# zhaodong-liu/GRAM

Measured on AMD Instinct MI355X. Metric: users/sec @ beam=20 top-20 gen, Beauty T5-base; Recall@5 parity, higher is better.
Workload: dtype f16x3

## Files before the change

gram_amd/csrc/enc_attn.hip:

```cpp
#include "common.h"
#include "prof.h"

#ifndef GRAM_ENC_ABL
#define GRAM_ENC_ABL 0
#endif

namespace {

__device__ __forceinline__ int kswz(int row, int chunk) { return row * 128 + ((chunk ^ ((row >> 1) & 7)) << 4); }
__device__ __forceinline__ int vtswz(int d, int key) { return d * 256 + ((((key >> 3) ^ (d & 15))) << 4) + (key & 7) * 2; }

template <int NKS, int S, bool ROWS>
__global__ __launch_bounds__(256) void enc_attn_kernel(const p16* __restrict__ qkv, const float* __restrict__ bias,
                                                       const uint8_t* __restrict__ mask, p16* __restrict__ out, int H,
                                                       long qkv_pstride, const int64_t* __restrict__ ids) {
  constexpr int L = 32 * NKS;
  using T = SplitTab<S>;
  extern __shared__ __attribute__((aligned(16))) char smem[];
  char* ks = smem;
  char* vts = smem + S * 128 * 128;
  float* bias_s = reinterpret_cast<float*>(smem + S * 2 * 128 * 128);
  float* mask_s = bias_s + 4 * 256;

  const int h = blockIdx.x, p = blockIdx.y;
  const int tid = threadIdx.x, lane = tid & 63, wave = tid >> 6;
  const int inner = H * 64;
  const size_t rs = (size_t)3 * inner;
  const p16* base = qkv + (ROWS ? (size_t)0 : (size_t)p * L * rs) + h * 64;
  long kvid[ROWS ? NKS : 1], qid[2];
  float bias_early = 0.f;
  uint32_t mask_early = 1;
  if constexpr (ROWS) {
    const int64_t* pid = ids + (size_t)p * L;
#pragma unroll
    for (int it = 0; it < NKS; ++it) kvid[it] = pid[(tid + it * 256) >> 3];
#pragma unroll
    for (int nt = 0; nt < 2; ++nt) qid[nt] = wave * 32 < L ? pid[wave * 32 + 16 * nt + (lane & 15)] : 0;
    if (tid < 255) bias_early = bias[h * 255 + tid];
    if (tid < L) mask_early = mask[(size_t)p * L + tid];
    asm volatile("" : "+v"(bias_early), "+v"(mask_early));
  }

#pragma unroll
  for (int pc = 0; pc < S; ++pc) {
    p16x8 kv[NKS], vv[NKS];
#pragma unroll
    for (int it = 0; it < NKS; ++it) {
      const int i = tid + it * 256, row = i >> 3, c = i & 7;
      const p16* src = base + pc * qkv_pstride + (size_t)(ROWS ? kvid[it] : row) * rs + c * 8;
      if constexpr ((GRAM_ENC_ABL & 8) != 0) {
        kv[it] = zero_bf16x8();
        vv[it] = zero_bf16x8();
        asm volatile("" : "+v"(kv[it]), "+v"(vv[it]));
      } else {
        kv[it] = ld_stream_b128(src + inner);
        vv[it] = ld_stream_b128(src + 2 * inner);
      }
    }
#pragma unroll
    for (int it = 0; it < NKS; ++it) {
      const int i = tid + it * 256, row = i >> 3, c = i & 7;
      *reinterpret_cast<p16x8*>(ks + pc * 128 * 128 + kswz(row, c)) = kv[it];
      if constexpr ((GRAM_ENC_ABL & 16) != 0) {
        *reinterpret_cast<p16x8*>(vts + pc * 64 * 256 + kswz(row, c)) = vv[it];
      } else {
#pragma unroll
        for (int e = 0; e < 8; ++e) *reinterpret_cast<p16*>(vts + pc * 64 * 256 + vtswz(c * 8 + e, row)) = vv[it][e];
      }
    }
  }
  if (tid < 255) {
    const float bv = ROWS ? bias_early : bias[h * 255 + tid];
#pragma unroll
    for (int r = 0; r < 4; ++r)
      if (tid >= r) bias_s[r * 256 + tid - r] = bv;
  }
  bool key_masked = false;
  if (tid < L) {
    key_masked = (ROWS ? mask_early : mask[(size_t)p * L + tid]) == 0;
    mask_s[tid] = key_masked ? 1.f : 0.f;
  }
  const bool any_masked = __syncthreads_or(key_masked) != 0;

  const int q0 = wave * 32;
  if (q0 >= L) return;
  const int c = lane & 15, g = lane >> 4;

  p16x8 qf[S][2][2];
#pragma unroll
  for (int pc = 0; pc < S; ++pc)
#pragma unroll
    for (int nt = 0; nt < 2; ++nt)
#pragma unroll
      for (int kd = 0; kd < 2; ++kd)
        if constexpr ((GRAM_ENC_ABL & 64) != 0) {
          qf[pc][nt][kd] = zero_bf16x8();
          asm volatile("" : "+v"(qf[pc][nt][kd]));
        } else {
          qf[pc][nt][kd] = ld_stream_b128(base + pc * qkv_pstride + (size_t)(ROWS ? qid[nt] : q0 + 16 * nt + c) * rs + 32 * kd + 8 * g);
        }

  f32x4 s[NKS][2][2];
#pragma unroll
  for (int k2 = 0; k2 < NKS; ++k2)
#pragma unroll
    for (int t = 0; t < 2; ++t) {
      const int key = 32 * k2 + 8 * (c >> 2) + 4 * t + (c & 3);
      p16x8 kf[S][2];
#pragma unroll
      for (int pc = 0; pc < S; ++pc) {
        kf[pc][0] = *reinterpret_cast<const p16x8*>(ks + pc * 128 * 128 + kswz(key, g));
        kf[pc][1] = *reinterpret_cast<const p16x8*>(ks + pc * 128 * 128 + kswz(key, 4 + g));
      }
#pragma unroll
      for (int nt = 0; nt < 2; ++nt) {
        const int idx0 = 32 * k2 + 8 * g + 4 * t + 127 - (q0 + 16 * nt + c), r = idx0 & 3;
        f32x4 a = *reinterpret_cast<const f32x4*>(bias_s + r * 256 + (idx0 - r));
        if constexpr ((GRAM_ENC_ABL & 1) != 0) {
          a[0] += (float)kf[0][0][0] + (float)qf[0][nt][0][0];
        } else {
#pragma unroll
          for (int pr = 0; pr < T::NP; ++pr) {
            a = mfma16(kf[T::A[pr]][0], qf[T::B[pr]][nt][0], a);
            a = mfma16(kf[T::A[pr]][1], qf[T::B[pr]][nt][1], a);
          }
        }
        s[k2][t][nt] = a;
      }
    }

  gram_sync();

  float mxq[2], l[2] = {0.f, 0.f};
#pragma unroll
  for (int nt = 0; nt < 2; ++nt) {
    float mx = GRAM_FMIN;
#pragma unroll
    for (int k2 = 0; k2 < NKS; ++k2)
#pragma unroll
      for (int t = 0; t < 2; ++t)
#pragma unroll
        for (int j = 0; j < 4; ++j) {
          float v = s[k2][t][nt][j];
          if (any_masked) {
            v = (mask_s[32 * k2 + 8 * g + 4 * t + j] != 0.f) ? GRAM_FMIN : v;
            s[k2][t][nt][j] = v;
          }
          mx = fmaxf(mx, v);
        }
    mx = fmaxf(mx, __shfl_xor(mx, 16, 64));
    mx = fmaxf(mx, __shfl_xor(mx, 32, 64));
    mxq[nt] = mx;
  }

  f32x4 o[4][2];
#pragma unroll
  for (int mt = 0; mt < 4; ++mt)
#pragma unroll
    for (int nt = 0; nt < 2; ++nt) o[mt][nt] = (f32x4){0.f, 0.f, 0.f, 0.f};
#pragma unroll
  for (int k2 = 0; k2 < NKS; ++k2) {
    p16x8 pf[S][2];
#pragma unroll
    for (int nt = 0; nt < 2; ++nt) {
      if constexpr ((GRAM_ENC_ABL & 2) != 0) {
        float t = 0.f;
#pragma unroll
        for (int tt = 0; tt < 2; ++tt)
#pragma unroll
          for (int j = 0; j < 4; ++j) t += s[k2][tt][nt][j];
        l[nt] += t;
        const uint32_t wv = __float_as_uint(t) & 0x3c003c00u;
        pf[0][nt] = __builtin_bit_cast(p16x8, make_uint4(wv, wv, wv, wv));
        if constexpr (S == 2) pf[S - 1][nt] = pf[0][nt];
      } else if constexpr (S == 2) {
        uint32_t w[2][4];
#pragma unroll
        for (int t = 0; t < 2; ++t)
#pragma unroll
          for (int j = 0; j < 4; j += 2) {
            const float e0 = __expf(s[k2][t][nt][j] - mxq[nt]), e1 = __expf(s[k2][t][nt][j + 1] - mxq[nt]);
            l[nt] += e0;
            l[nt] += e1;
            split2_pair(e0, e1, w[0][2 * t + (j >> 1)], w[1][2 * t + (j >> 1)]);
          }
        pf[0][nt] = __builtin_bit_cast(p16x8, make_uint4(w[0][0], w[0][1], w[0][2], w[0][3]));
        pf[1][nt] = __builtin_bit_cast(p16x8, make_uint4(w[1][0], w[1][1], w[1][2], w[1][3]));
      } else {
#pragma unroll
        for (int t = 0; t < 2; ++t)
#pragma unroll
          for (int j = 0; j < 4; ++j) {
            const float e = __expf(s[k2][t][nt][j] - mxq[nt]);
            l[nt] += e;
            pf[0][nt][4 * t + j] = (p16)e;
          }
      }
    }
#pragma unroll
    for (int mt = 0; mt < 4; ++mt) {
      const int d = 16 * mt + c;
      p16x8 vf[S];
#pragma unroll
      for (int pc = 0; pc < S; ++pc) vf[pc] = *reinterpret_cast<const p16x8*>(vts + pc * 64 * 256 + vtswz(d, 32 * k2 + 8 * g));
#pragma unroll
      for (int nt = 0; nt < 2; ++nt)
#pragma unroll
        for (int pr = 0; pr < T::NP; ++pr) {
          if constexpr ((GRAM_ENC_ABL & 4) != 0) o[mt][nt][0] += (float)vf[T::A[pr]][0] + (float)pf[T::B[pr]][nt][0];
          else o[mt][nt] = mfma16(vf[T::A[pr]], pf[T::B[pr]][nt], o[mt][nt]);
        }
    }
  }

  constexpr int RB = 128 * S, CPR = RB / 16;
  char* stage = ks + wave * (32 * RB);
#pragma unroll
  for (int nt = 0; nt < 2; ++nt) {
    float lt = l[nt];
    lt += __shfl_xor(lt, 16, 64);
    lt += __shfl_xor(lt, 32, 64);
    const float inv_l = 1.f / lt;
    const int ql = 16 * nt + c;
#pragma unroll
    for (int mt = 0; mt < 4; ++mt) {
      const f32x4 v = o[mt][nt] * inv_l;
      if constexpr (S == 2) {
        uint2 hi, lo;
        split2x4(v, hi, lo);
        const int ch = (mt >> 1) * 8 + (mt & 1) * 2 + (g >> 1);
        *reinterpret_cast<uint2*>(stage + ql * RB + (((ch) ^ (ql & 15)) << 4) + (g & 1) * 8) = hi;
        *reinterpret_cast<uint2*>(stage + ql * RB + (((ch + 4) ^ (ql & 15)) << 4) + (g & 1) * 8) = lo;
      } else {
        p16x4 r;
#pragma unroll
        for (int j = 0; j < 4; ++j) r[j] = (p16)v[j];
        const int ch = 2 * mt + (g >> 1);
        *reinterpret_cast<p16x4*>(stage + ql * RB + ((ch ^ (ql & 7)) << 4) + (g & 1) * 8) = r;
      }
    }
  }
  __builtin_amdgcn_wave_barrier();
  asm volatile("s_waitcnt lgkmcnt(0)" ::: "memory");
  char* obase = reinterpret_cast<char*>(out) + (((size_t)p * L + q0) * inner * S + (size_t)h * 64 * S) * sizeof(p16);
#pragma unroll
  for (int it = 0; it < RB / 32; ++it) {
    const int row = it * (64 / CPR) + lane / CPR, chunk = lane % CPR;
    const uint4 val = *reinterpret_cast<const uint4*>(stage + row * RB + ((chunk ^ (row & (CPR - 1))) << 4));
    if (!(GRAM_ENC_ABL & 32) || val.x == 0x12345678u)
      *reinterpret_cast<uint4*>(obase + (size_t)row * inner * S * sizeof(p16) + chunk * 16) = val;
  }
}

template <int S, bool ROWS>
int launch_enc(const void* qkv, const int64_t* ids, const float* bias, const uint8_t* mask, void* out, int P, int L, int H,
               long qkv_pstride, hipStream_t st) {
  const dim3 grid(H, P), block(256);
  constexpr int smem = S * 2 * 128 * 128 + (4 * 256 + 128) * 4;
  static bool attr_set = false;
  if (!attr_set && smem > 48 * 1024) {
    hipError_t e = hipFuncSetAttribute(reinterpret_cast<const void*>(enc_attn_kernel<1, S, ROWS>), hipFuncAttributeMaxDynamicSharedMemorySize, smem);
    if (e == hipSuccess) e = hipFuncSetAttribute(reinterpret_cast<const void*>(enc_attn_kernel<2, S, ROWS>), hipFuncAttributeMaxDynamicSharedMemorySize, smem);
    if (e == hipSuccess) e = hipFuncSetAttribute(reinterpret_cast<const void*>(enc_attn_kernel<3, S, ROWS>), hipFuncAttributeMaxDynamicSharedMemorySize, smem);
    if (e == hipSuccess) e = hipFuncSetAttribute(reinterpret_cast<const void*>(enc_attn_kernel<4, S, ROWS>), hipFuncAttributeMaxDynamicSharedMemorySize, smem);
    if (e != hipSuccess) return (int)e;
    attr_set = true;
  }
  switch (L / 32) {
    case 1: hipLaunchKernelGGL((enc_attn_kernel<1, S, ROWS>), grid, block, smem, st, (const p16*)qkv, bias, mask, (p16*)out, H, qkv_pstride, ids); break;
    case 2: hipLaunchKernelGGL((enc_attn_kernel<2, S, ROWS>), grid, block, smem, st, (const p16*)qkv, bias, mask, (p16*)out, H, qkv_pstride, ids); break;
    case 3: hipLaunchKernelGGL((enc_attn_kernel<3, S, ROWS>), grid, block, smem, st, (const p16*)qkv, bias, mask, (p16*)out, H, qkv_pstride, ids); break;
    default: hipLaunchKernelGGL((enc_attn_kernel<4, S, ROWS>), grid, block, smem, st, (const p16*)qkv, bias, mask, (p16*)out, H, qkv_pstride, ids); break;
  }
  GRAM_CHECK_LAUNCH();
  return 0;
}

}

extern "C" int gram_enc_self_attn(const void* qkv, const float* bias, const uint8_t* mask, void* out, int P, int L, int H,
                                  void* stream) {
  return gram_enc_self_attn_split(qkv, bias, mask, out, P, L, H, 1, 0, stream);
}

extern "C" int gram_enc_self_attn_split(const void* qkv, const float* bias, const uint8_t* mask, void* out, int P, int L, int H,
                                        int pieces, int64_t qkv_pstride, void* stream) {
  if (P < 1 || H < 1 || L < 32 || L > GRAM_MAX_PASSAGE_LEN || (L & 31) || pieces < 1 || pieces > GRAM_MAX_PIECES) return GRAM_E_ARG;
  if (pieces > 1 && qkv_pstride < (int64_t)P * L * 3 * H * 64) return GRAM_E_ARG;
  hipStream_t st = (hipStream_t)stream;
  gram_prof::Scope prof(GRAM_K_ENC_ATTN, st, 4.0 * P * H * L * L * 64 * (pieces == 2 ? 3 : 1));
  if (pieces == 2) return launch_enc<2, false>(qkv, nullptr, bias, mask, out, P, L, H, qkv_pstride, st);
  return launch_enc<1, false>(qkv, nullptr, bias, mask, out, P, L, H, qkv_pstride, st);
}

extern "C" int gram_enc_self_attn_rows_split(const void* qkv_table, const int64_t* ids, const float* bias, const uint8_t* mask,
                                             void* out, int P, int L, int H, int pieces, int64_t qkv_pstride, void* stream) {
  if (P < 1 || H < 1 || L < 32 || L > GRAM_MAX_PASSAGE_LEN || (L & 31) || pieces < 1 || pieces > GRAM_MAX_PIECES || !qkv_table || !ids)
    return GRAM_E_ARG;
  if (pieces > 1 && qkv_pstride < (int64_t)3 * H * 64) return GRAM_E_ARG;
  hipStream_t st = (hipStream_t)stream;
  gram_prof::Scope prof(GRAM_K_ENC_ATTN, st, 4.0 * P * H * L * L * 64 * (pieces == 2 ? 3 : 1));
  if (pieces == 2) return launch_enc<2, true>(qkv_table, ids, bias, mask, out, P, L, H, qkv_pstride, st);
  return launch_enc<1, true>(qkv_table, ids, bias, mask, out, P, L, H, qkv_pstride, st);
}
```

Baseline: 3209.

## Alias K and V^T shared memory to halve LDS and raise occupancy

```diff
diff --git a/gram_amd/csrc/enc_attn.hip b/gram_amd/csrc/enc_attn.hip
--- a/gram_amd/csrc/enc_attn.hip
+++ b/gram_amd/csrc/enc_attn.hip
@@ -10,20 +10,39 @@
 __device__ __forceinline__ int kswz(int row, int chunk) { return row * 128 + ((chunk ^ ((row >> 1) & 7)) << 4); }
 __device__ __forceinline__ int vtswz(int d, int key) { return d * 256 + ((((key >> 3) ^ (d & 15))) << 4) + (key & 7) * 2; }
 
+__device__ __forceinline__ void enc_split2_pair(float a, float b, uint32_t& hi, uint32_t& lo) {
+#ifdef GRAM_F16
+  typedef float f32x2_ __attribute__((ext_vector_type(2)));
+  typedef _Float16 h16x2_ __attribute__((ext_vector_type(2)));
+  const f32x2_ ab = {a, b};
+  hi = __builtin_bit_cast(uint32_t, __builtin_convertvector(ab, h16x2_));
+  asm("v_fma_mix_f32 %0, %1, -1.0, %0 op_sel_hi:[1,0,0]" : "+v"(a) : "v"(hi));
+  asm("v_fma_mix_f32 %0, %1, -1.0, %0 op_sel:[1,0,0] op_sel_hi:[1,0,0]" : "+v"(b) : "v"(hi));
+  const f32x2_ r = {a, b};
+  lo = __builtin_bit_cast(uint32_t, __builtin_convertvector(r, h16x2_));
+#else
+  split2_pair(a, b, hi, lo);
+#endif
+}
+__device__ __forceinline__ void enc_split2x4(f32x4 v, uint2& hi, uint2& lo) {
+  enc_split2_pair(v[0], v[1], hi.x, lo.x);
+  enc_split2_pair(v[2], v[3], hi.y, lo.y);
+}
+
 template <int NKS, int S, bool ROWS>
-__global__ __launch_bounds__(256) void enc_attn_kernel(const p16* __restrict__ qkv, const float* __restrict__ bias,
+__global__ __launch_bounds__(256, 3) void enc_attn_kernel(const p16* __restrict__ qkv, const float* __restrict__ bias,
                                                        const uint8_t* __restrict__ mask, p16* __restrict__ out, int H,
                                                        long qkv_pstride, const int64_t* __restrict__ ids) {
   constexpr int L = 32 * NKS;
   using T = SplitTab<S>;
   extern __shared__ __attribute__((aligned(16))) char smem[];
   char* ks = smem;
-  char* vts = smem + S * 128 * 128;
-  float* bias_s = reinterpret_cast<float*>(smem + S * 2 * 128 * 128);
+  char* vts = smem;
+  float* bias_s = reinterpret_cast<float*>(smem + S * 128 * 128);
   float* mask_s = bias_s + 4 * 256;
 
   const int h = blockIdx.x, p = blockIdx.y;
-  const int tid = threadIdx.x, lane = tid & 63, wave = tid >> 6;
+  const int tid = threadIdx.x, lane = tid & 63, wave = __builtin_amdgcn_readfirstlane(tid >> 6);
   const int inner = H * 64;
   const size_t rs = (size_t)3 * inner;
   const p16* base = qkv + (ROWS ? (size_t)0 : (size_t)p * L * rs) + h * 64;
@@ -41,34 +60,47 @@
     asm volatile("" : "+v"(bias_early), "+v"(mask_early));
   }
 
-#pragma unroll
-  for (int pc = 0; pc < S; ++pc) {
-    p16x8 kv[NKS], vv[NKS];
+  p16x8 kv[S][NKS], vv[S][NKS];
+  auto load_rows = [&](p16x8 (&dst)[S][NKS], const p16* from, int tid) {
+#pragma unroll
+    for (int pc = 0; pc < S; ++pc)
+#pragma unroll
+      for (int it = 0; it < NKS; ++it) {
+        const int i = tid + it * 256, row = i >> 3, c = i & 7;
+        const p16* src = from + pc * qkv_pstride;
+        if constexpr (ROWS) src += (size_t)kvid[it] * rs + c * 8;
+        else src += (uint32_t)row * (uint32_t)rs + c * 8;
+        if constexpr ((GRAM_ENC_ABL & 8) != 0) {
+          dst[pc][it] = zero_bf16x8();
+          asm volatile("" : "+v"(dst[pc][it]));
+        } else {
+          dst[pc][it] = ld_stream_b128(src);
+        }
+      }
+  };
+  load_rows(kv, base + inner, tid);
+  load_rows(vv, base + 2 * inner, tid);
+#pragma unroll
+  for (int pc = 0; pc < S; ++pc)
 #pragma unroll
     for (int it = 0; it < NKS; ++it) {
       const int i = tid + it * 256, row = i >> 3, c = i & 7;
-      const p16* src = base + pc * qkv_pstride + (size_t)(ROWS ? kvid[it] : row) * rs + c * 8;
-      if constexpr ((GRAM_ENC_ABL & 8) != 0) {
-        kv[it] = zero_bf16x8();
-        vv[it] = zero_bf16x8();
-        asm volatile("" : "+v"(kv[it]), "+v"(vv[it]));
-      } else {
-        kv[it] = ld_stream_b128(src + inner);
-        vv[it] = ld_stream_b128(src + 2 * inner);
-      }
-    }
-#pragma unroll
-    for (int it = 0; it < NKS; ++it) {
-      const int i = tid + it * 256, row = i >> 3, c = i & 7;
-      *reinterpret_cast<p16x8*>(ks + pc * 128 * 128 + kswz(row, c)) = kv[it];
-      if constexpr ((GRAM_ENC_ABL & 16) != 0) {
-        *reinterpret_cast<p16x8*>(vts + pc * 64 * 256 + kswz(row, c)) = vv[it];
-      } else {
-#pragma unroll
-        for (int e = 0; e < 8; ++e) *reinterpret_cast<p16*>(vts + pc * 64 * 256 + vtswz(c * 8 + e, row)) = vv[it][e];
-      }
-    }
-  }
+      *reinterpret_cast<p16x8*>(ks + pc * 128 * 128 + kswz(row, c)) = kv[pc][it];
+    }
+  auto scatter_v = [&](int tid) {
+#pragma unroll
+    for (int pc = 0; pc < S; ++pc)
+#pragma unroll
+      for (int it = 0; it < NKS; ++it) {
+        const int i = tid + it * 256, row = i >> 3, c = i & 7;
+        if constexpr ((GRAM_ENC_ABL & 16) != 0) {
+          *reinterpret_cast<p16x8*>(vts + pc * 64 * 256 + kswz(row, c)) = vv[pc][it];
+        } else {
+#pragma unroll
+          for (int e = 0; e < 8; ++e) *reinterpret_cast<p16*>(vts + pc * 64 * 256 + vtswz(c * 8 + e, row)) = vv[pc][it][e];
+        }
+      }
+  };
   if (tid < 255) {
     const float bv = ROWS ? bias_early : bias[h * 255 + tid];
 #pragma unroll
@@ -81,55 +113,71 @@
     mask_s[tid] = key_masked ? 1.f : 0.f;
   }
   const bool any_masked = __syncthreads_or(key_masked) != 0;
+  gram_chaos_point();
 
   const int q0 = wave * 32;
-  if (q0 >= L) return;
-  const int c = lane & 15, g = lane >> 4;
-
-  p16x8 qf[S][2][2];
-#pragma unroll
-  for (int pc = 0; pc < S; ++pc)
-#pragma unroll
-    for (int nt = 0; nt < 2; ++nt)
-#pragma unroll
-      for (int kd = 0; kd < 2; ++kd)
-        if constexpr ((GRAM_ENC_ABL & 64) != 0) {
-          qf[pc][nt][kd] = zero_bf16x8();
-          asm volatile("" : "+v"(qf[pc][nt][kd]));
-        } else {
-          qf[pc][nt][kd] = ld_stream_b128(base + pc * qkv_pstride + (size_t)(ROWS ? qid[nt] : q0 + 16 * nt + c) * rs + 32 * kd + 8 * g);
-        }
-
+  if (NKS < 4 && q0 >= L) {
+    gram_sync();
+    scatter_v(tid);
+    gram_sync();
+    gram_sync();
+    return;
+  }
   f32x4 s[NKS][2][2];
-#pragma unroll
-  for (int k2 = 0; k2 < NKS; ++k2)
-#pragma unroll
-    for (int t = 0; t < 2; ++t) {
-      const int key = 32 * k2 + 8 * (c >> 2) + 4 * t + (c & 3);
-      p16x8 kf[S][2];
-#pragma unroll
-      for (int pc = 0; pc < S; ++pc) {
-        kf[pc][0] = *reinterpret_cast<const p16x8*>(ks + pc * 128 * 128 + kswz(key, g));
-        kf[pc][1] = *reinterpret_cast<const p16x8*>(ks + pc * 128 * 128 + kswz(key, 4 + g));
-      }
-#pragma unroll
-      for (int nt = 0; nt < 2; ++nt) {
-        const int idx0 = 32 * k2 + 8 * g + 4 * t + 127 - (q0 + 16 * nt + c), r = idx0 & 3;
-        f32x4 a = *reinterpret_cast<const f32x4*>(bias_s + r * 256 + (idx0 - r));
-        if constexpr ((GRAM_ENC_ABL & 1) != 0) {
-          a[0] += (float)kf[0][0][0] + (float)qf[0][nt][0][0];
-        } else {
-#pragma unroll
-          for (int pr = 0; pr < T::NP; ++pr) {
-            a = mfma16(kf[T::A[pr]][0], qf[T::B[pr]][nt][0], a);
-            a = mfma16(kf[T::A[pr]][1], qf[T::B[pr]][nt][1], a);
-          }
-        }
-        s[k2][t][nt] = a;
-      }
-    }
-
+  {
+    const int c = lane & 15, g = lane >> 4;
+    p16x8 qf[S][2][2];
+#pragma unroll
+    for (int pc = 0; pc < S; ++pc)
+#pragma unroll
+      for (int nt = 0; nt < 2; ++nt)
+#pragma unroll
+        for (int kd = 0; kd < 2; ++kd)
+          if constexpr ((GRAM_ENC_ABL & 64) != 0) {
+            qf[pc][nt][kd] = zero_bf16x8();
+            asm volatile("" : "+v"(qf[pc][nt][kd]));
+          } else {
+            qf[pc][nt][kd] = ld_stream_b128(base + pc * qkv_pstride + (ROWS ? (size_t)qid[nt] * rs : (size_t)((uint32_t)(q0 + 16 * nt + c) * (uint32_t)rs)) + 32 * kd + 8 * g);
+          }
+
+#pragma unroll
+    for (int k2 = 0; k2 < NKS; ++k2)
+#pragma unroll
+      for (int t = 0; t < 2; ++t) {
+        const int key = 32 * k2 + 8 * (c >> 2) + 4 * t + (c & 3);
+        p16x8 kf[S][2];
+#pragma unroll
+        for (int pc = 0; pc < S; ++pc) {
+          kf[pc][0] = *reinterpret_cast<const p16x8*>(ks + pc * 128 * 128 + kswz(key, g));
+          kf[pc][1] = *reinterpret_cast<const p16x8*>(ks + pc * 128 * 128 + kswz(key, 4 + g));
+        }
+#pragma unroll
+        for (int nt = 0; nt < 2; ++nt) {
+          const int idx0 = 32 * k2 + 8 * g + 4 * t + 127 - (q0 + 16 * nt + c), r = idx0 & 3;
+          f32x4 a = *reinterpret_cast<const f32x4*>(bias_s + r * 256 + (idx0 - r));
+          if constexpr ((GRAM_ENC_ABL & 1) != 0) {
+            a[0] += (float)kf[0][0][0] + (float)qf[0][nt][0][0];
+          } else {
+#pragma unroll
+            for (int pr = 0; pr < T::NP; ++pr) {
+              a = mfma16(kf[T::A[pr]][0], qf[T::B[pr]][nt][0], a);
+              a = mfma16(kf[T::A[pr]][1], qf[T::B[pr]][nt][1], a);
+            }
+          }
+          s[k2][t][nt] = a;
+        }
+      }
+  }
   gram_sync();
+  {
+    int t = tid;
+    asm volatile("" : "+v"(t)::"memory");
+    scatter_v(t);
+  }
+  gram_sync();
+  int ln = lane;
+  asm volatile("" : "+v"(ln));
+  const int c = ln & 15, g = ln >> 4;
 
   float mxq[2], l[2] = {0.f, 0.f};
 #pragma unroll
@@ -182,7 +230,7 @@
             const float e0 = __expf(s[k2][t][nt][j] - mxq[nt]), e1 = __expf(s[k2][t][nt][j + 1] - mxq[nt]);
             l[nt] += e0;
             l[nt] += e1;
-            split2_pair(e0, e1, w[0][2 * t + (j >> 1)], w[1][2 * t + (j >> 1)]);
+            enc_split2_pair(e0, e1, w[0][2 * t + (j >> 1)], w[1][2 * t + (j >> 1)]);
           }
         pf[0][nt] = __builtin_bit_cast(p16x8, make_uint4(w[0][0], w[0][1], w[0][2], w[0][3]));
         pf[1][nt] = __builtin_bit_cast(p16x8, make_uint4(w[1][0], w[1][1], w[1][2], w[1][3]));
@@ -213,42 +261,49 @@
     }
   }
 
-  constexpr int RB = 128 * S, CPR = RB / 16;
-  char* stage = ks + wave * (32 * RB);
-#pragma unroll
-  for (int nt = 0; nt < 2; ++nt) {
-    float lt = l[nt];
-    lt += __shfl_xor(lt, 16, 64);
-    lt += __shfl_xor(lt, 32, 64);
-    const float inv_l = 1.f / lt;
-    const int ql = 16 * nt + c;
-#pragma unroll
-    for (int mt = 0; mt < 4; ++mt) {
-      const f32x4 v = o[mt][nt] * inv_l;
-      if constexpr (S == 2) {
-        uint2 hi, lo;
-        split2x4(v, hi, lo);
-        const int ch = (mt >> 1) * 8 + (mt & 1) * 2 + (g >> 1);
-        *reinterpret_cast<uint2*>(stage + ql * RB + (((ch) ^ (ql & 15)) << 4) + (g & 1) * 8) = hi;
-        *reinterpret_cast<uint2*>(stage + ql * RB + (((ch + 4) ^ (ql & 15)) << 4) + (g & 1) * 8) = lo;
-      } else {
-        p16x4 r;
-#pragma unroll
-        for (int j = 0; j < 4; ++j) r[j] = (p16)v[j];
-        const int ch = 2 * mt + (g >> 1);
-        *reinterpret_cast<p16x4*>(stage + ql * RB + ((ch ^ (ql & 7)) << 4) + (g & 1) * 8) = r;
-      }
-    }
-  }
-  __builtin_amdgcn_wave_barrier();
-  asm volatile("s_waitcnt lgkmcnt(0)" ::: "memory");
-  char* obase = reinterpret_cast<char*>(out) + (((size_t)p * L + q0) * inner * S + (size_t)h * 64 * S) * sizeof(p16);
-#pragma unroll
-  for (int it = 0; it < RB / 32; ++it) {
-    const int row = it * (64 / CPR) + lane / CPR, chunk = lane % CPR;
-    const uint4 val = *reinterpret_cast<const uint4*>(stage + row * RB + ((chunk ^ (row & (CPR - 1))) << 4));
-    if (!(GRAM_ENC_ABL & 32) || val.x == 0x12345678u)
-      *reinterpret_cast<uint4*>(obase + (size_t)row * inner * S * sizeof(p16) + chunk * 16) = val;
+  gram_sync();
+
+  {
+    constexpr int RB = 128 * S, CPR = RB / 16;
+    int lo = ln;
+    asm volatile("" : "+v"(lo));
+    const int lane = lo, c = lo & 15, g = lo >> 4;
+    char* stage = ks + wave * (32 * RB);
+#pragma unroll
+    for (int nt = 0; nt < 2; ++nt) {
+      float lt = l[nt];
+      lt += __shfl_xor(lt, 16, 64);
+      lt += __shfl_xor(lt, 32, 64);
+      const float inv_l = 1.f / lt;
+      const int ql = 16 * nt + c;
+#pragma unroll
+      for (int mt = 0; mt < 4; ++mt) {
+        const f32x4 v = o[mt][nt] * inv_l;
+        if constexpr (S == 2) {
+          uint2 hi, lo;
+          enc_split2x4(v, hi, lo);
+          const int ch = (mt >> 1) * 8 + (mt & 1) * 2 + (g >> 1);
+          *reinterpret_cast<uint2*>(stage + ql * RB + (((ch) ^ (ql & 15)) << 4) + (g & 1) * 8) = hi;
+          *reinterpret_cast<uint2*>(stage + ql * RB + (((ch + 4) ^ (ql & 15)) << 4) + (g & 1) * 8) = lo;
+        } else {
+          p16x4 r;
+#pragma unroll
+          for (int j = 0; j < 4; ++j) r[j] = (p16)v[j];
+          const int ch = 2 * mt + (g >> 1);
+          *reinterpret_cast<p16x4*>(stage + ql * RB + ((ch ^ (ql & 7)) << 4) + (g & 1) * 8) = r;
+        }
+      }
+    }
+    __builtin_amdgcn_wave_barrier();
+    asm volatile("s_waitcnt lgkmcnt(0)" ::: "memory");
+    char* obase = reinterpret_cast<char*>(out) + (((size_t)p * L + q0) * inner * S + (size_t)h * 64 * S) * sizeof(p16);
+#pragma unroll
+    for (int it = 0; it < RB / 32; ++it) {
+      const int row = it * (64 / CPR) + lane / CPR, chunk = lane % CPR;
+      const uint4 val = *reinterpret_cast<const uint4*>(stage + row * RB + ((chunk ^ (row & (CPR - 1))) << 4));
+      if (!(GRAM_ENC_ABL & 32) || val.x == 0x12345678u)
+        *reinterpret_cast<uint4*>(obase + (size_t)row * inner * S * sizeof(p16) + chunk * 16) = val;
+    }
   }
 }
 
@@ -256,7 +311,7 @@
 int launch_enc(const void* qkv, const int64_t* ids, const float* bias, const uint8_t* mask, void* out, int P, int L, int H,
                long qkv_pstride, hipStream_t st) {
   const dim3 grid(H, P), block(256);
-  constexpr int smem = S * 2 * 128 * 128 + (4 * 256 + 128) * 4;
+  constexpr int smem = S * 128 * 128 + (4 * 256 + 128) * 4;
   static bool attr_set = false;
   if (!attr_set && smem > 48 * 1024) {
     hipError_t e = hipFuncSetAttribute(reinterpret_cast<const void*>(enc_attn_kernel<1, S, ROWS>), hipFuncAttributeMaxDynamicSharedMemorySize, smem);
```

New measurement: 3217 (median of 3 runs). No clear change (+0.2%).
